# karfly/learnable-triangulation-pytorch

Hardware: NVIDIA H100
Metric: volumetric samples/sec (4-view 384x384, 64^3 grid) (higher is better)
Workload: dtype fp16x3 (split-fp16 operands, 3 wgmma products per term, fp32 accumulate)

## Files before the change

### learnable-triangulation-pytorch_b200/csrc/conv_tc.cu

```cuda
#include "tc_common.cuh"
#include "conv_tc_params.cuh"
#include <stdlib.h>
#include <string.h>

namespace lt {

constexpr int kTcThreads = 384;

struct TcUnit {
  int m, n0, z, q_begin, nchunks;
};
__device__ __forceinline__ TcUnit tc_unit(const TcParams& p, int u, int m_tiles, int nchunks_all) {
  TcUnit w;
  const int n = u % p.n_tiles;
  u /= p.n_tiles;
  w.m = u % m_tiles;
  w.z = u / m_tiles;
  w.n0 = n * p.Nt;
  w.q_begin = (int)(((long)w.z * nchunks_all) / p.splits);
  w.nchunks = (int)(((long)(w.z + 1) * nchunks_all) / p.splits) - w.q_begin;
  return w;
}
__device__ __forceinline__ void tc_tile_origin(const TcParams& p, int t, int& ow0, int& oh0, int& od0, int& nb0) {
  ow0 = (t % p.tw) * p.bw; t /= p.tw;
  oh0 = (t % p.th) * p.bh; t /= p.th;
  od0 = (t % p.td) * p.bd;
  nb0 = (t / p.td) * p.bn;
}

constexpr int kSlabBytes = 128 * 128;
__host__ __device__ constexpr int tc_epi_bytes(int nt, int splits) { return (nt >= 32 && splits == 1) ? nt / 32 * kSlabBytes : 0; }

__device__ __forceinline__ void epi_slab(const TcParams& p, int co, int& g, int& c) {
  g = p.n_maps > 1 ? co / p.oc : 0;
  const int ch = co - g * p.oc;
  c = p.out_format == LT_FMT_F32 ? ch : 2 * ch;
}

__device__ __forceinline__ uint32_t sw128(int row, int b) {
  return (uint32_t)(row * 128 + ((((b >> 4) ^ row) & 7) << 4) + (b & 15));
}

template <int NT>
__global__ void __launch_bounds__(kTcThreads, 1) conv_tc_kernel(const __grid_constant__ CUtensorMap tmA,
                                                                const __grid_constant__ CUtensorMap tmB,
                                                                const __grid_constant__ TcEpiMaps tmE, const TcParams p) {
  extern __shared__ uint8_t smem_raw[];
  uint8_t* smem = reinterpret_cast<uint8_t*>((reinterpret_cast<uintptr_t>(smem_raw) + 1023) & ~(uintptr_t)1023);
  constexpr int kStage = kATileBytes + NT * 128;
  const int epi_bytes = tc_epi_bytes(NT, p.splits);
  const bool staged = epi_bytes > 0;
  uint8_t* ebuf = smem + (size_t)p.stages * kStage;
  uint64_t* full = reinterpret_cast<uint64_t*>(ebuf + epi_bytes);
  uint64_t* empty = full + p.stages;
  uint64_t* efull = empty + p.stages;
  uint64_t* edone = efull + 1;

  const int wg = __shfl_sync(0xffffffffu, (int)(threadIdx.x >> 7), 0);
  const int lane = threadIdx.x & 31;
  const int m_tiles = p.tw * p.th * p.td * p.tn;
  const int units = m_tiles * p.n_tiles * p.splits;
  const int nchunks_all = p.KD * p.KH * p.KW * p.CB;

  if (threadIdx.x == 0) {
    for (int s = 0; s < p.stages; ++s) { mbar_init(&full[s], 1); mbar_init(&empty[s], 2); }
    mbar_init(efull, 1);
    mbar_init(edone, 256);
    fence_barrier_init();
    prefetch_tmap(&tmA);
    prefetch_tmap(&tmB);
  }
  __syncthreads();

  if (wg == 0) {
    regs_release_producer();
    if (staged && threadIdx.x == 32) {
      uint32_t eph = 0;
      for (int u = blockIdx.x; u < units; u += gridDim.x) {
        const TcUnit w = tc_unit(p, u, m_tiles, nchunks_all);
        int ow0, oh0, od0, nb0;
        tc_tile_origin(p, w.m, ow0, oh0, od0, nb0);
        bulk_wait_read0();
        if (p.residual != LT_RES_NONE) {
          mbar_expect_tx(efull, (uint32_t)epi_bytes);
          for (int sl = 0; sl < NT / 32; ++sl) {
            int g, c;
            epi_slab(p, w.n0 + 32 * sl, g, c);
            tma_load_5d(ebuf + sl * kSlabBytes, &tmE.res[g], efull, c, ow0, oh0, od0, nb0);
          }
        } else {
          mbar_arrive_local(efull);
        }
        mbar_wait(edone, eph);
        eph ^= 1u;
        for (int sl = 0; sl < NT / 32; ++sl) {
          int g, c;
          epi_slab(p, w.n0 + 32 * sl, g, c);
          tma_store_5d(&tmE.out[g], ebuf + sl * kSlabBytes, c, ow0, oh0, od0, nb0);
        }
        bulk_commit();
      }
      bulk_wait0();
    }
    if (threadIdx.x < 32) {
      int s = 0;
      uint32_t ph = 0;
      for (int u = blockIdx.x; u < units; u += gridDim.x) {
        const TcUnit w = tc_unit(p, u, m_tiles, nchunks_all);
        int ow0, oh0, od0, nb0;
        tc_tile_origin(p, w.m, ow0, oh0, od0, nb0);
        int tap = w.q_begin / p.CB, cb = w.q_begin - tap * p.CB;
        int kw = tap % p.KW, kh = (tap / p.KW) % p.KH, kd = tap / (p.KW * p.KH);
        const int ax = ow0 * p.sw - p.pw, ay = oh0 * p.sh - p.ph, az = od0 * p.sd - p.pd, bn0 = w.n0 * p.b_nmul;
        for (int q = 0, qa = w.q_begin; q < w.nchunks; ++q, ++qa) {
          mbar_wait(&empty[s], ph ^ 1u);
          uint8_t* a_dst = smem + (size_t)s * kStage;
          if (elect_one()) {
            mbar_expect_tx(&full[s], (uint32_t)kStage);
            tma_load_5d(a_dst, &tmA, &full[s], cb * 64, ax + kw, ay + kh, az + kd, nb0);
            tma_load_2d(a_dst + kATileBytes, &tmB, &full[s], qa * p.b_step0, qa * p.b_step1 + bn0);
          }
          __syncwarp();
          if (++cb == p.CB) { cb = 0; if (++kw == p.KW) { kw = 0; if (++kh == p.KH) { kh = 0; ++kd; } } }
          if (++s == p.stages) { s = 0; ph ^= 1u; }
        }
      }
    }
    return;
  }

  regs_claim_consumer();
  const int g = wg - 1;
  float d1[NT / 2], d2[NT / 2];
#pragma unroll
  for (int i = 0; i < NT / 2; ++i) { d1[i] = 0.f; d2[i] = 0.f; }
  const int r0 = g * 64 + ((threadIdx.x >> 5) & 3) * 16 + (lane >> 2);
  const int c2 = 2 * (lane & 3);
  const uint32_t ring0 = smem_u32(smem);
  int s = 0;
  uint32_t ph = 0, eph = 0;
  for (int u = blockIdx.x; u < units; u += gridDim.x) {
    const TcUnit w = tc_unit(p, u, m_tiles, nchunks_all);
    int prev = -1;
    for (int q = 0; q < w.nchunks; ++q) {
      mbar_wait(&full[s], ph);
      const uint32_t a_addr = ring0 + (uint32_t)(s * kStage) + (uint32_t)(g * 64 * 128);
      const uint32_t b_addr = ring0 + (uint32_t)(s * kStage) + kATileBytes;
      const uint64_t ad = make_sw128_desc(a_addr), bd = make_sw128_desc(b_addr);
      const uint32_t acc = (q == 0) ? 0u : 1u;
      wg_fence();
      if (p.terms == 3) {
        wgmma_f16<NT>(d1, ad, bd, acc);
        wgmma_f16<NT>(d1, ad + 2, bd + 2, 1u);
        wgmma_f16<NT>(d2, ad, bd + 4, acc);
        wgmma_f16<NT>(d2, ad + 2, bd + 6, 1u);
        wgmma_f16<NT>(d2, ad + 4, bd, 1u);
        wgmma_f16<NT>(d2, ad + 6, bd + 2, 1u);
      } else if (p.terms == 1) {
        wgmma_f16<NT>(d1, ad, bd, acc);
        wgmma_f16<NT>(d1, ad + 2, bd + 2, 1u);
      } else {
        wgmma_f16<NT>(d1, ad, bd, acc);
        wgmma_f16<NT>(d1, ad + 2, bd + 2, 1u);
        wgmma_f16<NT>(d1, ad + 4, bd + 4, 1u);
        wgmma_f16<NT>(d1, ad + 6, bd + 6, 1u);
      }
      wg_commit();
      wg_wait<1>();
      if (prev >= 0 && (threadIdx.x & 127) == 0) mbar_arrive_local(&empty[prev]);
      prev = s;
      if (++s == p.stages) { s = 0; ph ^= 1u; }
    }
    wg_wait<0>();
    if (prev >= 0 && (threadIdx.x & 127) == 0) mbar_arrive_local(&empty[prev]);
    wg_fence_regs(d1);
    wg_fence_regs(d2);

    if (p.splits > 1) {
#pragma unroll
      for (int h = 0; h < 2; ++h) {
        float* wrow = p.ws + (((size_t)w.z * m_tiles + w.m) * 128 + r0 + 8 * h) * p.ws_ld + w.n0;
#pragma unroll
        for (int i = 0; i < NT / 8; ++i) {
          const int k = 4 * i + 2 * h;
          const float v0 = (p.terms == 3) ? fmaf(d2[k], kLoInv, d1[k]) : d1[k];
          const float v1 = (p.terms == 3) ? fmaf(d2[k + 1], kLoInv, d1[k + 1]) : d1[k + 1];
          *reinterpret_cast<float2*>(wrow + 8 * i + c2) = make_float2(v0, v1);
        }
      }
      continue;
    }
    if constexpr (NT >= 32) {
      mbar_wait(efull, eph);
      eph ^= 1u;
      const uint32_t e0 = smem_u32(ebuf);
      auto fc_ok = [&](int co) {
        int ch;
        long pix;
        epilogue_target(p, co, 0, ch, pix);
        return ch < p.FC;
      };
      float2 sc = make_float2(0.f, 0.f), sh = sc;
      if (fc_ok(w.n0 + c2)) {
        sc = __ldg(reinterpret_cast<const float2*>(p.scale + w.n0 + c2));
        sh = __ldg(reinterpret_cast<const float2*>(p.shift + w.n0 + c2));
      }
#pragma unroll
      for (int i = 0; i < NT / 8; ++i) {
        const int co = w.n0 + 8 * i + c2;
        const bool ok = fc_ok(co);
        float2 sc_next = sc, sh_next = sh;
        if (i + 1 < NT / 8 && fc_ok(co + 8)) {
          sc_next = __ldg(reinterpret_cast<const float2*>(p.scale + co + 8));
          sh_next = __ldg(reinterpret_cast<const float2*>(p.shift + co + 8));
        }
        const uint32_t slab = e0 + (uint32_t)((i >> 2) * kSlabBytes);
        const int cc = 8 * (i & 3) + c2;
#pragma unroll
        for (int h = 0; h < 2 && ok; ++h) {
          const int row = r0 + 8 * h;
          const int k = 4 * i + 2 * h;
          float v0 = (p.terms == 3) ? fmaf(d2[k], kLoInv, d1[k]) : d1[k];
          float v1 = (p.terms == 3) ? fmaf(d2[k + 1], kLoInv, d1[k + 1]) : d1[k + 1];
          v0 = fmaf(v0, sc.x, sh.x);
          v1 = fmaf(v1, sc.y, sh.y);
          if (p.out_format == LT_FMT_F32) {
            const uint32_t a = slab + sw128(row, 4 * cc);
            float2 r = make_float2(0.f, 0.f);
            if (p.residual != LT_RES_NONE) r = lds_f2(a);
            if (p.residual == LT_RES_BEFORE_RELU) { v0 += r.x; v1 += r.y; }
            if (p.relu) { v0 = fmaxf(v0, 0.f); v1 = fmaxf(v1, 0.f); }
            if (p.residual == LT_RES_AFTER_RELU) { v0 += r.x; v1 += r.y; }
            sts_f2(a, make_float2(v0, v1));
          } else {
            const uint32_t ahi = slab + sw128(row, 2 * cc), alo = slab + sw128(row, 64 + 2 * cc);
            float2 r = make_float2(0.f, 0.f);
            if (p.residual != LT_RES_NONE) {
              const uint32_t rh = lds32(ahi), rl = lds32(alo);
              const float2 a = __half22float2(*reinterpret_cast<const __half2*>(&rh));
              const float2 b = __half22float2(*reinterpret_cast<const __half2*>(&rl));
              r = make_float2(fmaf(b.x, kLoInv, a.x), fmaf(b.y, kLoInv, a.y));
            }
            if (p.residual == LT_RES_BEFORE_RELU) { v0 += r.x; v1 += r.y; }
            if (p.relu) { v0 = fmaxf(v0, 0.f); v1 = fmaxf(v1, 0.f); }
            if (p.residual == LT_RES_AFTER_RELU) { v0 += r.x; v1 += r.y; }
            uint32_t hi2, lo2;
            split_s32x2(v0, v1, hi2, lo2);
            sts32(ahi, hi2);
            sts32(alo, lo2);
          }
        }
        sc = sc_next;
        sh = sh_next;
      }
      fence_proxy_async();
      mbar_arrive_local(edone);
    } else {
      int ow0, oh0, od0, nb0;
      tc_tile_origin(p, w.m, ow0, oh0, od0, nb0);
#pragma unroll
      for (int h = 0; h < 2; ++h) {
        int r_ = r0 + 8 * h;
        const int dw = r_ % p.bw; r_ /= p.bw;
        const int dh = r_ % p.bh; r_ /= p.bh;
        const int dd = r_ % p.bd; r_ /= p.bd;
        const int ow = ow0 + dw, oh = oh0 + dh, od = od0 + dd, nb = nb0 + r_;
        if (!(ow < p.OW && oh < p.OH && od < p.OD && nb < p.N)) continue;
        const long opix = (((long)nb * p.FD + (od * p.osd + p.ood)) * p.FH + (oh * p.osh + p.ooh)) * p.FW + (ow * p.osw + p.oow);
        conv_epilogue_row<NT>(p, d1, d2, h, opix, w.n0, c2);
      }
    }
  }
}

typedef CUresult (*EncodeTiledFn)(CUtensorMap*, CUtensorMapDataType, cuuint32_t, void*, const cuuint64_t*, const cuuint64_t*,
                                  const cuuint32_t*, const cuuint32_t*, CUtensorMapInterleave, CUtensorMapSwizzle,
                                  CUtensorMapL2promotion, CUtensorMapFloatOOBfill);

static EncodeTiledFn encode_fn() {
  static EncodeTiledFn fn = nullptr;
  if (!fn) {
    void* ptr = nullptr;
    cudaDriverEntryPointQueryResult qres;
    if (cudaGetDriverEntryPoint("cuTensorMapEncodeTiled", &ptr, cudaEnableDefault, &qres) == cudaSuccess &&
        qres == cudaDriverEntryPointSuccess)
      fn = reinterpret_cast<EncodeTiledFn>(ptr);
  }
  return fn;
}

struct MapKey {
  const void* base;
  int rank, swizzle, f32;
  uint64_t dims[5], strides[4];
  uint32_t box[5], es[5];
};
struct MapSlot {
  bool used = false;
  MapKey key;
  CUtensorMap map;
};

int make_map(CUtensorMap* map, const void* base, int rank, const uint64_t* dims, const uint64_t* strides_bytes,
             const uint32_t* box, const uint32_t* estrides, int swizzle128, int f32) {
  EncodeTiledFn fn = encode_fn();
  if (!fn) return fail(LT_ERR_CUDA, "cuTensorMapEncodeTiled entry point not available");
  MapKey key;
  memset(&key, 0, sizeof(key));
  key.base = base; key.rank = rank; key.swizzle = swizzle128; key.f32 = f32;
  for (int i = 0; i < rank; ++i) { key.dims[i] = dims[i]; key.box[i] = box[i]; key.es[i] = estrides ? estrides[i] : 1; }
  for (int i = 0; i + 1 < rank; ++i) key.strides[i] = strides_bytes[i];
  uint64_t h = 1469598103934665603ull;
  const unsigned char* kb = reinterpret_cast<const unsigned char*>(&key);
  for (size_t i = 0; i < sizeof(key); ++i) { h ^= kb[i]; h *= 1099511628211ull; }
  static thread_local MapSlot cache[256];
  MapSlot& slot = cache[(h ^ (h >> 29)) & 255];
  if (slot.used && memcmp(&slot.key, &key, sizeof(key)) == 0) {
    *map = slot.map;
    return LT_OK;
  }
  cuuint64_t gd[5], gs[4];
  cuuint32_t bx[5], es[5];
  for (int i = 0; i < rank; ++i) { gd[i] = dims[i]; bx[i] = box[i]; es[i] = estrides ? estrides[i] : 1; }
  for (int i = 0; i + 1 < rank; ++i) gs[i] = strides_bytes[i];
  CUresult r = fn(map, f32 ? CU_TENSOR_MAP_DATA_TYPE_FLOAT32 : CU_TENSOR_MAP_DATA_TYPE_FLOAT16, (cuuint32_t)rank, const_cast<void*>(base), gd, gs, bx, es,
                  CU_TENSOR_MAP_INTERLEAVE_NONE,
                  swizzle128 == 1 ? CU_TENSOR_MAP_SWIZZLE_128B : (swizzle128 == 2 ? CU_TENSOR_MAP_SWIZZLE_64B : CU_TENSOR_MAP_SWIZZLE_NONE),
                  CU_TENSOR_MAP_L2_PROMOTION_L2_128B, CU_TENSOR_MAP_FLOAT_OOB_FILL_NONE);
  if (r != CUDA_SUCCESS) return fail(LT_ERR_CUDA, "cuTensorMapEncodeTiled failed with CUresult %d", (int)r);
  slot.used = true;
  slot.key = key;
  slot.map = *map;
  return LT_OK;
}

static int pow2_ceil(int v) { int p = 1; while (p < v) p <<= 1; return p; }

static void pick_box(int OW, int OH, int OD, int N, int* box) {
  double best = 1e300;
  for (int bw = 1; bw <= 128; bw <<= 1)
    for (int bh = 1; bw * bh <= 128; bh <<= 1)
      for (int bd = 1; bw * bh * bd <= 128; bd <<= 1) {
        const int bn = 128 / (bw * bh * bd);
        if (bw > pow2_ceil(OW) || bh > pow2_ceil(OH) || bd > pow2_ceil(OD) || bn > pow2_ceil(N)) continue;
        const double padded = (double)ceil_div(OW, bw) * bw * ceil_div(OH, bh) * bh * (double)ceil_div(OD, bd) * bd * ceil_div(N, bn) * bn;
        const double score = padded * (1.0 + 1e-3 / bw);
        if (score < best) { best = score; box[0] = bw; box[1] = bh; box[2] = bd; box[3] = bn; }
      }
  if (best == 1e300) { box[0] = pow2_ceil(OW) > 128 ? 128 : pow2_ceil(OW); box[1] = box[2] = 1; box[3] = 128 / box[0]; }
}

__global__ void __launch_bounds__(256) splitk_reduce_kernel(const TcParams p, long m_tiles, int coutp) {
  const int c4 = coutp >> 2;
  const long total = m_tiles * 128 * c4;
  for (long i = (long)blockIdx.x * blockDim.x + threadIdx.x; i < total; i += (long)gridDim.x * blockDim.x) {
    const int co = (int)(i % c4) * 4;
    const long tr = i / c4;
    const int row = (int)(tr % 128);
    long t = tr / 128;
    const int twi = (int)(t % p.tw); t /= p.tw;
    const int thi = (int)(t % p.th); t /= p.th;
    const int tdi = (int)(t % p.td); t /= p.td;
    const int tni = (int)t;
    int r_ = row;
    const int dw = r_ % p.bw; r_ /= p.bw;
    const int dh = r_ % p.bh; r_ /= p.bh;
    const int dd = r_ % p.bd; r_ /= p.bd;
    const int ow = twi * p.bw + dw, oh = thi * p.bh + dh, od = tdi * p.bd + dd, nb = tni * p.bn + r_;
    if (!(ow < p.OW && oh < p.OH && od < p.OD && nb < p.N) || co >= p.FC) continue;
    const long opix = (((long)nb * p.FD + (od * p.osd + p.ood)) * p.FH + (oh * p.osh + p.ooh)) * p.FW + (ow * p.osw + p.oow);
    float4 a = make_float4(0.f, 0.f, 0.f, 0.f);
    for (int z = 0; z < p.splits; ++z) {
      const float4 v = *reinterpret_cast<const float4*>(p.ws + ((size_t)z * m_tiles * 128 + tr) * p.ws_ld + co);
      a.x += v.x; a.y += v.y; a.z += v.z; a.w += v.w;
    }
    const float4 sc = __ldg(reinterpret_cast<const float4*>(p.scale + co));
    const float4 sh = __ldg(reinterpret_cast<const float4*>(p.shift + co));
    float4 o = make_float4(fmaf(a.x, sc.x, sh.x), fmaf(a.y, sc.y, sh.y), fmaf(a.z, sc.z, sh.z), fmaf(a.w, sc.w, sh.w));
    float4 rr = make_float4(0.f, 0.f, 0.f, 0.f);
    if (p.residual != LT_RES_NONE) {
      if (p.out_format == LT_FMT_F32) rr = *reinterpret_cast<const float4*>(reinterpret_cast<const float*>(p.res) + opix * p.FC + co);
      else rr = load_s32x4(reinterpret_cast<const sh_t*>(p.res) + opix * 2 * p.FC, co);
    }
    if (p.residual == LT_RES_BEFORE_RELU) { o.x += rr.x; o.y += rr.y; o.z += rr.z; o.w += rr.w; }
    if (p.relu) { o.x = fmaxf(o.x, 0.f); o.y = fmaxf(o.y, 0.f); o.z = fmaxf(o.z, 0.f); o.w = fmaxf(o.w, 0.f); }
    if (p.residual == LT_RES_AFTER_RELU) { o.x += rr.x; o.y += rr.y; o.z += rr.z; o.w += rr.w; }
    if (p.out_format == LT_FMT_F32) *reinterpret_cast<float4*>(reinterpret_cast<float*>(p.out) + opix * p.FC + co) = o;
    else store_s32x4(reinterpret_cast<sh_t*>(p.out) + opix * 2 * p.FC, co, o);
  }
}

static int out_groups(const lt_conv_desc* d) {
  const int g = (d->ogd > 1 ? d->ogd : 1) * (d->ogh > 1 ? d->ogh : 1) * (d->ogw > 1 ? d->ogw : 1);
  return g;
}

static int pick_nt(int CoutP) {
  for (int nt = 128; nt > 16; nt >>= 1)
    if (CoutP % nt == 0) return nt;
  return 16;
}

template <int NT>
static int launch_nt(const CUtensorMap& tmA, const CUtensorMap& tmB, const TcEpiMaps& tmE, const TcParams& p, dim3 grid, size_t smem,
                     cudaStream_t st) {
  static DeviceOnce configured;
  if (configured.first()) {
    cudaError_t e = cudaFuncSetAttribute(conv_tc_kernel<NT>, cudaFuncAttributeMaxDynamicSharedMemorySize, (int)(227 * 1024));
    if (e != cudaSuccess) return fail(LT_ERR_CUDA, "conv_tc: cudaFuncSetAttribute: %s", cudaGetErrorString(e));
  }
  conv_tc_kernel<NT><<<grid, kTcThreads, smem, st>>>(tmA, tmB, tmE, p);
  cudaError_t e = cudaGetLastError();
  if (e != cudaSuccess) return fail(LT_ERR_CUDA, "conv_tc_kernel: %s", cudaGetErrorString(e));
  return LT_OK;
}

static double tc_model_clocks(long tiles, int chunks, int nt, int splits, int sm) {
  const long units = tiles * splits;
  const long grid = units < sm ? units : sm;
  const long waves = (units + grid - 1) / grid;
  const double chunk = fmax(12.0 * 64.0 * nt / 128.0, (kATileBytes + nt * 128.0) / 30.0);
  const double epilogue = 128.0 * nt * 4.0 / 30.0;
  double t = (double)waves * ((double)ceil_div(chunks, splits) * chunk + epilogue);
  if (splits > 1) t += 7000.0 + (double)tiles * 128 * nt * 4.0 * (splits + 2) / 1500.0;
  return t;
}

static void tc_plan(long m_tiles, int n_tiles, int nt, int chunks, int terms, int n_maps, int splitk, size_t ws_bytes, int sm,
                    int* splits_out, int* grid_out) {
  const long tiles = m_tiles * n_tiles;
  int best = 1;
  if (splitk && terms != 0 && n_maps == 1) {
    const size_t per_split = (size_t)tiles * 128 * nt * sizeof(float);
    double best_t = tc_model_clocks(tiles, chunks, nt, 1, sm);
    for (int s = 2; s <= chunks / 4 && (size_t)s * per_split <= ws_bytes; ++s) {
      const double t = tc_model_clocks(tiles, chunks, nt, s, sm);
      if (t < best_t) { best_t = t; best = s; }
    }
  }
  const long units = tiles * best;
  *splits_out = best;
  *grid_out = (int)(units < sm ? units : sm);
}

static int group_extent(int n, int F, int off, int ph, int os) {
  const int e = (F - off - ph + os - 1) / os;
  return e < n ? e : n;
}

static int make_epi_maps(const TcParams& p, TcEpiMaps* m) {
  const int f32 = p.out_format == LT_FMT_F32;
  const uint64_t rowb = (uint64_t)p.FC * 4;
  const uint64_t str[4] = {rowb * p.osw, rowb * p.FW * p.osh, rowb * p.FW * p.FH * p.osd, rowb * p.FW * p.FH * p.FD};
  const uint32_t bx[5] = {f32 ? 32u : 64u, (uint32_t)p.bw, (uint32_t)p.bh, (uint32_t)p.bd, (uint32_t)p.bn};
  for (int g = 0; g < p.n_maps; ++g) {
    const int ga = g / (p.gh * p.gw), gb = (g / p.gw) % p.gh, gc = g % p.gw;
    const int ew = group_extent(p.OW, p.FW, p.oow, gc, p.osw), eh = group_extent(p.OH, p.FH, p.ooh, gb, p.osh),
              ed = group_extent(p.OD, p.FD, p.ood, ga, p.osd);
    LT_REQUIRE(ew > 0 && eh > 0 && ed > 0, "conv_tc: output group %d lies outside the %dx%dx%d output tensor", g, p.FD, p.FH, p.FW);
    const uint64_t dims[5] = {(uint64_t)(f32 ? p.FC : 2 * p.FC), (uint64_t)ew, (uint64_t)eh, (uint64_t)ed, (uint64_t)p.N};
    const long pix0 = ((long)(p.ood + ga) * p.FH + p.ooh + gb) * p.FW + p.oow + gc;
    int rc = make_map(&m->out[g], static_cast<const uint8_t*>(p.out) + pix0 * rowb, 5, dims, str, bx, nullptr, 1, f32);
    if (rc) return rc;
    if (p.residual == LT_RES_NONE) continue;
    rc = make_map(&m->res[g], static_cast<const uint8_t*>(p.res) + pix0 * rowb, 5, dims, str, bx, nullptr, 1, f32);
    if (rc) return rc;
  }
  return LT_OK;
}

constexpr int kTcSmemBudget = 224 * 1024;

static int launch_tc(const CUtensorMap& tmA, const CUtensorMap& tmB, TcParams& p, int n_tiles, cudaStream_t st, void* ws = nullptr,
                     size_t ws_bytes = 0) {
  const long m_tiles = (long)p.tw * p.th * p.td * p.tn;
  int splits, grid;
  tc_plan(m_tiles, n_tiles, p.Nt, p.KD * p.KH * p.KW * p.CB, p.terms, p.n_maps, ws ? opts().tc_splitk : 0, ws_bytes, sm_count(),
          &splits, &grid);
  p.splits = splits;
  p.ws = reinterpret_cast<float*>(ws);
  p.ws_ld = n_tiles * p.Nt;
  p.n_tiles = n_tiles;
  const int stage_bytes = kATileBytes + p.Nt * 128;
  const int epi_bytes = tc_epi_bytes(p.Nt, splits);
  int stages = (kTcSmemBudget - epi_bytes) / stage_bytes;
  if (stages > 8) stages = 8;
  p.stages = stages;
  const size_t smem = (size_t)stages * stage_bytes + epi_bytes + (2 * stages + 2) * 8 + 1024;
  TcEpiMaps tmE{};
  int rc;
  if (epi_bytes) {
    rc = make_epi_maps(p, &tmE);
    if (rc) return rc;
  }
  switch (p.Nt) {
    case 128: rc = launch_nt<128>(tmA, tmB, tmE, p, dim3(grid), smem, st); break;
    case 64: rc = launch_nt<64>(tmA, tmB, tmE, p, dim3(grid), smem, st); break;
    case 32: rc = launch_nt<32>(tmA, tmB, tmE, p, dim3(grid), smem, st); break;
    case 16: rc = launch_nt<16>(tmA, tmB, tmE, p, dim3(grid), smem, st); break;
    default: return fail(LT_ERR_INVALID, "conv_tc: unsupported N tile %d", p.Nt);
  }
  if (rc) return rc;
  if (splits > 1) {
    const long total = m_tiles * 128 * (p.ws_ld / 4);
    long blocks = (total + 255) / 256;
    if (blocks > 4L * sm_count()) blocks = 4L * sm_count();
    splitk_reduce_kernel<<<(unsigned)blocks, 256, 0, st>>>(p, m_tiles, p.ws_ld);
    cudaError_t e = cudaGetLastError();
    if (e != cudaSuccess) return fail(LT_ERR_CUDA, "splitk_reduce_kernel: %s", cudaGetErrorString(e));
  }
  return LT_OK;
}

void fill_params(const lt_conv_desc* d, TcParams& p, int CB, int CoutP, int Nt, int terms, const float* scale, const float* shift,
                        const void* residual, void* out) {
  p.OW = d->OW; p.OH = d->OH; p.OD = d->OD; p.N = d->N;
  int box[4];
  pick_box(d->OW, d->OH, d->OD, d->N, box);
  p.bw = box[0]; p.bh = box[1]; p.bd = box[2]; p.bn = box[3];
  p.tw = ceil_div(d->OW, p.bw); p.th = ceil_div(d->OH, p.bh); p.td = ceil_div(d->OD, p.bd); p.tn = ceil_div(d->N, p.bn);
  p.KW = d->KW; p.KH = d->KH; p.KD = d->KD; p.pw = d->pw; p.ph = d->ph; p.pd = d->pd;
  p.sw = d->sw; p.sh = d->sh; p.sd = d->sd;
  p.CB = CB; p.b_step0 = 0; p.b_step1 = CoutP; p.b_nmul = 1; p.Nt = Nt; p.terms = terms;
  p.FC = d->FC; p.FD = d->FD; p.FH = d->FH; p.FW = d->FW;
  p.osd = d->osd; p.osh = d->osh; p.osw = d->osw; p.ood = d->ood; p.ooh = d->ooh; p.oow = d->oow;
  p.relu = d->relu; p.residual = d->residual; p.out_format = d->out_format;
  p.scale = scale; p.shift = shift; p.res = residual; p.out = out;
  p.splits = 1; p.ws = nullptr; p.ws_ld = 0; p.stages = 0; p.n_tiles = 1;
  p.n_maps = out_groups(d);
  p.oc = p.n_maps > 1 ? d->Cout / p.n_maps : CoutP;
  p.gh = d->ogh > 1 ? d->ogh : 1; p.gw = d->ogw > 1 ? d->ogw : 1;
}

int make_in_map(CUtensorMap* tmA, const lt_conv_desc* d, int bw, int bh, int bd, int bn, const void* in) {
  const uint64_t rowb = (uint64_t)d->Cin * 2 * 2;
  const uint64_t dims[5] = {(uint64_t)d->Cin * 2, (uint64_t)d->IW, (uint64_t)d->IH, (uint64_t)d->ID, (uint64_t)d->N};
  const uint64_t str[4] = {rowb, rowb * d->IW, rowb * d->IW * d->IH, rowb * d->IW * d->IH * d->ID};
  const uint32_t es[5] = {1, (uint32_t)d->sw, (uint32_t)d->sh, (uint32_t)d->sd, 1};
  uint32_t bx[5] = {64, (uint32_t)bw, (uint32_t)bh, (uint32_t)bd, (uint32_t)bn};
  for (int i = 1; i <= 3; ++i) bx[i] = (bx[i] - 1) * es[i] + 1;
  LT_REQUIRE(bx[1] <= 256 && bx[2] <= 256 && bx[3] <= 256, "conv_tc: strided box exceeds 256");
  return make_map(tmA, in, 5, dims, str, bx, es, 1);
}

static bool groups_ok(const lt_conv_desc* d, int CoutP) {
  const int G = out_groups(d);
  return d->Cout % G == 0 && (d->Cout / G) % 32 == 0 && d->Cout / G == d->FC && CoutP == d->Cout && G <= kMaxOutMaps;
}

int conv_tc_fwd_terms(const lt_conv_desc* d, const void* in, const void* weight, const float* scale, const float* shift,
                      const void* residual, void* out, int terms, void* stream) {
  LT_REQUIRE(d->in_format == LT_FMT_S32, "conv_tc: input must be split-fp16");
  LT_REQUIRE(d->Cin % 32 == 0, "conv_tc: Cin=%d must be a multiple of 32", d->Cin);
  LT_REQUIRE(d->FC % 4 == 0 && (d->out_format == LT_FMT_F32 || d->FC % 32 == 0), "conv_tc: bad output channel stride %d", d->FC);
  LT_REQUIRE((reinterpret_cast<uintptr_t>(out) | reinterpret_cast<uintptr_t>(residual)) % 16 == 0,
             "conv_tc: out and residual must be 16-byte aligned (TMA global addresses)");
  const int CoutP = (d->Cout + 15) & ~15;
  const int CB = d->Cin / 32;
  const int taps = d->KD * d->KH * d->KW;
  const int Nt = pick_nt(CoutP);
  TcParams p;
  fill_params(d, p, CB, CoutP, Nt, terms, scale, shift, residual, out);
  if (p.n_maps > 1)
    LT_REQUIRE(groups_ok(d, CoutP), "conv_tc: grouped output needs Cout / groups == FC, a multiple of 32");
  CUtensorMap tmA, tmB;
  int rc = make_in_map(&tmA, d, p.bw, p.bh, p.bd, p.bn, in);
  if (rc) return rc;
  {
    const uint64_t dims[2] = {64, (uint64_t)taps * CB * CoutP};
    const uint64_t str[1] = {128};
    const uint32_t bx[2] = {64, (uint32_t)Nt};
    rc = make_map(&tmB, weight, 2, dims, str, bx, nullptr, 1);
    if (rc) return rc;
  }
  return launch_tc(tmA, tmB, p, CoutP / Nt, (cudaStream_t)stream, d->workspace, d->workspace_bytes);
}

__global__ void __launch_bounds__(256) pack_weights_kernel(const float* __restrict__ w, sh_t* __restrict__ out,
                                                           int taps, int Cin, int Cout, int CoutP) {
  const int CB = Cin / 32;
  const long total = (long)taps * CB * CoutP * 32;
  for (long i = (long)blockIdx.x * blockDim.x + threadIdx.x; i < total; i += (long)gridDim.x * blockDim.x) {
    const int j = (int)(i % 32);
    long r = i / 32;
    const int n = (int)(r % CoutP); r /= CoutP;
    const int cb = (int)(r % CB);
    const int tap = (int)(r / CB);
    const float v = (n < Cout) ? w[((long)tap * Cin + cb * 32 + j) * Cout + n] : 0.0f;
    sh_t hi, lo;
    split_s32(v, hi, lo);
    sh_t* rowp = out + ((((long)tap * CB + cb) * CoutP + n) << 6);
    rowp[j] = hi;
    rowp[32 + j] = lo;
  }
}

__global__ void ones_zeros_kernel(float* ones, float* zeros, int n) {
  const int i = blockIdx.x * blockDim.x + threadIdx.x;
  if (i < n) { ones[i] = 1.0f; zeros[i] = 0.0f; }
}

}

using namespace lt;

extern "C" int lt_conv_tc_plan(const lt_conv_desc* d, int sm_count, int splitk, lt_conv_tc_launch_plan* plan) {
  LT_REQUIRE(d && plan && sm_count > 0, "conv_tc_plan: bad arguments");
  LT_REQUIRE(d->Cin % 32 == 0 && d->Cout > 0, "conv_tc_plan: Cin=%d must be a multiple of 32", d->Cin);
  const int CoutP = (d->Cout + 15) & ~15;
  int box[4];
  pick_box(d->OW, d->OH, d->OD, d->N, box);
  plan->nt = pick_nt(CoutP);
  plan->m_tiles = ceil_div(d->OW, box[0]) * ceil_div(d->OH, box[1]) * ceil_div(d->OD, box[2]) * ceil_div(d->N, box[3]);
  plan->n_tiles = CoutP / plan->nt;
  plan->chunks = d->KD * d->KH * d->KW * (d->Cin / 32);
  tc_plan(plan->m_tiles, plan->n_tiles, plan->nt, plan->chunks, 3, out_groups(d), d->workspace ? splitk : 0, d->workspace_bytes,
          sm_count, &plan->splits, &plan->grid);
  return LT_OK;
}

extern "C" size_t lt_conv_tc_weight_bytes(int taps, int Cin, int Cout) {
  const int CoutP = (Cout + 15) & ~15;
  return (size_t)taps * (Cin / 32) * CoutP * 128;
}

extern "C" int lt_conv_tc_pack_weights(const float* w, void* packed, int taps, int Cin, int Cout, void* stream) {
  LT_REQUIRE(w && packed, "conv_tc_pack_weights: null pointer");
  LT_REQUIRE(Cin % 32 == 0 && taps > 0 && Cout > 0, "conv_tc_pack_weights: bad sizes");
  const int CoutP = (Cout + 15) & ~15;
  const long total = (long)taps * (Cin / 32) * CoutP * 32;
  long blocks = (total + 255) / 256;
  if (blocks > 65535) blocks = 65535;
  pack_weights_kernel<<<(unsigned)blocks, 256, 0, (cudaStream_t)stream>>>(w, reinterpret_cast<sh_t*>(packed), taps, Cin, Cout, CoutP);
  LT_CHECK_LAUNCH("pack_weights_kernel");
  return LT_OK;
}

extern "C" int lt_tc_gemm_selftest(const void* a, const void* b, float* d, int M, int N, int K, int variant, void* stream) {
  LT_REQUIRE(a && b && d, "tc_gemm_selftest: null pointer");
  LT_REQUIRE(M > 0 && N % 16 == 0 && N >= 16 && K % 64 == 0, "tc_gemm_selftest: need N %% 16 == 0, K %% 64 == 0");
  (void)variant;
  const int Nt = pick_nt(N);
  float* ones = d + (size_t)M * N;
  float* zeros = ones + N;
  ones_zeros_kernel<<<ceil_div(N, 256), 256, 0, (cudaStream_t)stream>>>(ones, zeros, N);
  TcParams p;
  p.OW = M; p.OH = 1; p.OD = 1; p.N = 1;
  p.bw = 128; p.bh = 1; p.bd = 1; p.bn = 1;
  p.tw = ceil_div(M, 128); p.th = 1; p.td = 1; p.tn = 1;
  p.KW = p.KH = p.KD = 1; p.pw = p.ph = p.pd = 0; p.sw = p.sh = p.sd = 1;
  p.CB = K / 64; p.b_step0 = 64; p.b_step1 = 0; p.b_nmul = 1; p.Nt = Nt; p.terms = 0;
  p.FC = N; p.FD = 1; p.FH = 1; p.FW = M; p.osd = p.osh = p.osw = 1; p.ood = p.ooh = p.oow = 0;
  p.relu = 0; p.residual = LT_RES_NONE; p.out_format = LT_FMT_F32;
  p.scale = ones; p.shift = zeros; p.res = nullptr; p.out = d;
  p.n_maps = 1; p.oc = N; p.gh = p.gw = 1;
  p.splits = 1; p.ws = nullptr; p.ws_ld = 0; p.n_tiles = 1;
  CUtensorMap tmA, tmB;
  {
    const uint64_t dims[5] = {(uint64_t)K, (uint64_t)M, 1, 1, 1};
    const uint64_t str[4] = {(uint64_t)K * 2, (uint64_t)K * 2 * M, (uint64_t)K * 2 * M, (uint64_t)K * 2 * M};
    const uint32_t bx[5] = {64, 128, 1, 1, 1};
    int rc = make_map(&tmA, a, 5, dims, str, bx, nullptr, 1);
    if (rc) return rc;
  }
  {
    const uint64_t dims[2] = {(uint64_t)K, (uint64_t)N};
    const uint64_t str[1] = {(uint64_t)K * 2};
    const uint32_t bx[2] = {64, (uint32_t)Nt};
    int rc = make_map(&tmB, b, 2, dims, str, bx, nullptr, 1);
    if (rc) return rc;
  }
  return launch_tc(tmA, tmB, p, N / Nt, (cudaStream_t)stream);
}
```

### learnable-triangulation-pytorch_b200/csrc/conv_tc_params.cuh

```cuda
#pragma once
#include "tc_common.cuh"

namespace lt {

struct TcParams {
  int OW, OH, OD, N;
  int bw, bh, bd, bn;
  int tw, th, td, tn;
  int KW, KH, KD, pw, ph, pd;
  int sw, sh, sd;
  int CB;
  int b_step0, b_step1;
  int b_nmul;
  int Nt, stages, terms;
  int FC, FD, FH, FW, osd, osh, osw, ood, ooh, oow, relu, residual, out_format;
  const float* scale;
  const float* shift;
  const void* res;
  void* out;
  int splits, ws_ld;
  float* ws;
  int n_tiles;
  int oc, n_maps;
  int gh, gw;
};

constexpr int kMaxOutMaps = 8;

struct TcEpiMaps {
  CUtensorMap out[kMaxOutMaps];
  CUtensorMap res[kMaxOutMaps];
};

constexpr int kATileBytes = 128 * 128;

__device__ __forceinline__ void epilogue_target(const TcParams& p, int co, long opix, int& ch, long& pix) {
  ch = co;
  pix = opix;
  if (p.n_maps > 1) {
    const int mi = ch / p.oc;
    ch -= mi * p.oc;
    pix += ((long)(mi / (p.gh * p.gw)) * p.FH + (mi / p.gw) % p.gh) * p.FW + mi % p.gw;
  }
}

template <int NT>
__device__ __forceinline__ float2 epilogue_residual(const TcParams& p, int ch, long pix) {
  if (p.residual == LT_RES_NONE || ch >= p.FC) return make_float2(0.f, 0.f);
  if (p.out_format == LT_FMT_F32) return *reinterpret_cast<const float2*>(reinterpret_cast<const float*>(p.res) + pix * p.FC + ch);
  const sh_t* rp = reinterpret_cast<const sh_t*>(p.res) + pix * 2 * p.FC + s32_off(ch);
  const float2 a = __half22float2(*reinterpret_cast<const __half2*>(rp));
  const float2 b = __half22float2(*reinterpret_cast<const __half2*>(rp + 32));
  return make_float2(fmaf(b.x, kLoInv, a.x), fmaf(b.y, kLoInv, a.y));
}

template <int NT>
__device__ __forceinline__ void conv_epilogue_row(const TcParams& p, const float (&d1)[NT / 2], const float (&d2)[NT / 2], int h,
                                                  long opix, int n0, int c2) {
  static_assert(NT <= 32, "wider tiles would not hold the hoisted residual beside their accumulators");
  float2 rr[NT / 8];
#pragma unroll
  for (int i = 0; i < NT / 8; ++i) {
    int ch;
    long pix;
    epilogue_target(p, n0 + 8 * i + c2, opix, ch, pix);
    rr[i] = epilogue_residual<NT>(p, ch, pix);
  }
#pragma unroll
  for (int i = 0; i < NT / 8; ++i) {
    const int k = 4 * i + 2 * h;
    const int co = n0 + 8 * i + c2;
    int ch;
    long pix;
    epilogue_target(p, co, opix, ch, pix);
    if (ch >= p.FC) continue;
    float v0 = (p.terms == 3) ? fmaf(d2[k], kLoInv, d1[k]) : d1[k];
    float v1 = (p.terms == 3) ? fmaf(d2[k + 1], kLoInv, d1[k + 1]) : d1[k + 1];
    const float2 sc = __ldg(reinterpret_cast<const float2*>(p.scale + co));
    const float2 sh = __ldg(reinterpret_cast<const float2*>(p.shift + co));
    v0 = fmaf(v0, sc.x, sh.x);
    v1 = fmaf(v1, sc.y, sh.y);
    const float2 r = rr[i];
    if (p.residual == LT_RES_BEFORE_RELU) { v0 += r.x; v1 += r.y; }
    if (p.relu) { v0 = fmaxf(v0, 0.f); v1 = fmaxf(v1, 0.f); }
    if (p.residual == LT_RES_AFTER_RELU) { v0 += r.x; v1 += r.y; }
    if (p.out_format == LT_FMT_F32) {
      *reinterpret_cast<float2*>(reinterpret_cast<float*>(p.out) + pix * p.FC + ch) = make_float2(v0, v1);
    } else {
      uint32_t hi2, lo2;
      split_s32x2(v0, v1, hi2, lo2);
      sh_t* op = reinterpret_cast<sh_t*>(p.out) + pix * 2 * p.FC + s32_off(ch);
      *reinterpret_cast<uint32_t*>(op) = hi2;
      *reinterpret_cast<uint32_t*>(op + 32) = lo2;
    }
  }
}

void fill_params(const lt_conv_desc* d, TcParams& p, int CB, int CoutP, int Nt, int terms, const float* scale, const float* shift,
                 const void* residual, void* out);
int make_in_map(CUtensorMap* tmA, const lt_conv_desc* d, int bw, int bh, int bd, int bn, const void* in);

}
```

Measured before the change: 193.9.

## Double-buffer the TMA epilogue staging buffer for short-K conv units

```diff
diff --git a/learnable-triangulation-pytorch_b200/csrc/conv_tc.cu b/learnable-triangulation-pytorch_b200/csrc/conv_tc.cu
--- a/learnable-triangulation-pytorch_b200/csrc/conv_tc.cu
+++ b/learnable-triangulation-pytorch_b200/csrc/conv_tc.cu
@@ -50,11 +50,12 @@
   constexpr int kStage = kATileBytes + NT * 128;
   const int epi_bytes = tc_epi_bytes(NT, p.splits);
   const bool staged = epi_bytes > 0;
+  const int nbuf = p.ebufs;
   uint8_t* ebuf = smem + (size_t)p.stages * kStage;
-  uint64_t* full = reinterpret_cast<uint64_t*>(ebuf + epi_bytes);
+  uint64_t* full = reinterpret_cast<uint64_t*>(ebuf + (size_t)nbuf * epi_bytes);
   uint64_t* empty = full + p.stages;
   uint64_t* efull = empty + p.stages;
-  uint64_t* edone = efull + 1;
+  uint64_t* edone = efull + 2;
 
   const int wg = __shfl_sync(0xffffffffu, (int)(threadIdx.x >> 7), 0);
   const int lane = threadIdx.x & 31;
@@ -64,8 +65,7 @@
 
   if (threadIdx.x == 0) {
     for (int s = 0; s < p.stages; ++s) { mbar_init(&full[s], 1); mbar_init(&empty[s], 2); }
-    mbar_init(efull, 1);
-    mbar_init(edone, 256);
+    for (int b = 0; b < 2; ++b) { mbar_init(&efull[b], 1); mbar_init(&edone[b], 256); }
     fence_barrier_init();
     prefetch_tmap(&tmA);
     prefetch_tmap(&tmB);
@@ -75,30 +75,44 @@
   if (wg == 0) {
     regs_release_producer();
     if (staged && threadIdx.x == 32) {
-      uint32_t eph = 0;
-      for (int u = blockIdx.x; u < units; u += gridDim.x) {
+      auto load_residual = [&](int u, int b) {
         const TcUnit w = tc_unit(p, u, m_tiles, nchunks_all);
         int ow0, oh0, od0, nb0;
         tc_tile_origin(p, w.m, ow0, oh0, od0, nb0);
-        bulk_wait_read0();
+        uint8_t* eb = ebuf + (size_t)b * epi_bytes;
         if (p.residual != LT_RES_NONE) {
-          mbar_expect_tx(efull, (uint32_t)epi_bytes);
+          mbar_expect_tx(&efull[b], (uint32_t)epi_bytes);
           for (int sl = 0; sl < NT / 32; ++sl) {
             int g, c;
             epi_slab(p, w.n0 + 32 * sl, g, c);
-            tma_load_5d(ebuf + sl * kSlabBytes, &tmE.res[g], efull, c, ow0, oh0, od0, nb0);
+            tma_load_5d(eb + sl * kSlabBytes, &tmE.res[g], &efull[b], c, ow0, oh0, od0, nb0);
           }
         } else {
-          mbar_arrive_local(efull);
-        }
-        mbar_wait(edone, eph);
-        eph ^= 1u;
+          mbar_arrive_local(&efull[b]);
+        }
+      };
+      if ((int)blockIdx.x < units) load_residual(blockIdx.x, 0);
+      int i = 0;
+      for (int u = blockIdx.x; u < units; u += gridDim.x, ++i) {
+        const int b = i % nbuf, next = u + gridDim.x;
+        if (nbuf == 2 && next < units) {
+          bulk_wait_read0();
+          load_residual(next, b ^ 1);
+        }
+        const TcUnit w = tc_unit(p, u, m_tiles, nchunks_all);
+        int ow0, oh0, od0, nb0;
+        tc_tile_origin(p, w.m, ow0, oh0, od0, nb0);
+        mbar_wait(&edone[b], (uint32_t)(i / nbuf) & 1u);
         for (int sl = 0; sl < NT / 32; ++sl) {
           int g, c;
           epi_slab(p, w.n0 + 32 * sl, g, c);
-          tma_store_5d(&tmE.out[g], ebuf + sl * kSlabBytes, c, ow0, oh0, od0, nb0);
+          tma_store_5d(&tmE.out[g], ebuf + (size_t)b * epi_bytes + sl * kSlabBytes, c, ow0, oh0, od0, nb0);
         }
         bulk_commit();
+        if (nbuf == 1 && next < units) {
+          bulk_wait_read0();
+          load_residual(next, 0);
+        }
       }
       bulk_wait0();
     }
@@ -138,8 +152,8 @@
   const int c2 = 2 * (lane & 3);
   const uint32_t ring0 = smem_u32(smem);
   int s = 0;
-  uint32_t ph = 0, eph = 0;
-  for (int u = blockIdx.x; u < units; u += gridDim.x) {
+  uint32_t ph = 0;
+  for (int u = blockIdx.x, i = 0; u < units; u += gridDim.x, ++i) {
     const TcUnit w = tc_unit(p, u, m_tiles, nchunks_all);
     int prev = -1;
     for (int q = 0; q < w.nchunks; ++q) {
@@ -191,9 +205,9 @@
       continue;
     }
     if constexpr (NT >= 32) {
-      mbar_wait(efull, eph);
-      eph ^= 1u;
-      const uint32_t e0 = smem_u32(ebuf);
+      const int b = i % nbuf;
+      mbar_wait(&efull[b], (uint32_t)(i / nbuf) & 1u);
+      const uint32_t e0 = smem_u32(ebuf + (size_t)b * epi_bytes);
       auto fc_ok = [&](int co) {
         int ch;
         long pix;
@@ -254,7 +268,7 @@
         sh = sh_next;
       }
       fence_proxy_async();
-      mbar_arrive_local(edone);
+      mbar_arrive_local(&edone[b]);
     } else {
       int ow0, oh0, od0, nb0;
       tc_tile_origin(p, w.m, ow0, oh0, od0, nb0);
@@ -470,6 +484,7 @@
 }
 
 constexpr int kTcSmemBudget = 224 * 1024;
+constexpr int kTcShortK = 4;
 
 static int launch_tc(const CUtensorMap& tmA, const CUtensorMap& tmB, TcParams& p, int n_tiles, cudaStream_t st, void* ws = nullptr,
                      size_t ws_bytes = 0) {
@@ -483,10 +498,12 @@
   p.n_tiles = n_tiles;
   const int stage_bytes = kATileBytes + p.Nt * 128;
   const int epi_bytes = tc_epi_bytes(p.Nt, splits);
-  int stages = (kTcSmemBudget - epi_bytes) / stage_bytes;
+  const int unit_chunks = ceil_div(p.KD * p.KH * p.KW * p.CB, splits);
+  p.ebufs = (epi_bytes && unit_chunks <= kTcShortK && (kTcSmemBudget - 2 * epi_bytes) / stage_bytes >= 3) ? 2 : 1;
+  int stages = (kTcSmemBudget - p.ebufs * epi_bytes) / stage_bytes;
   if (stages > 8) stages = 8;
   p.stages = stages;
-  const size_t smem = (size_t)stages * stage_bytes + epi_bytes + (2 * stages + 2) * 8 + 1024;
+  const size_t smem = (size_t)stages * stage_bytes + (size_t)p.ebufs * epi_bytes + (2 * stages + 4) * 8 + 1024;
   TcEpiMaps tmE{};
   int rc;
   if (epi_bytes) {
@@ -526,7 +543,7 @@
   p.osd = d->osd; p.osh = d->osh; p.osw = d->osw; p.ood = d->ood; p.ooh = d->ooh; p.oow = d->oow;
   p.relu = d->relu; p.residual = d->residual; p.out_format = d->out_format;
   p.scale = scale; p.shift = shift; p.res = residual; p.out = out;
-  p.splits = 1; p.ws = nullptr; p.ws_ld = 0; p.stages = 0; p.n_tiles = 1;
+  p.splits = 1; p.ws = nullptr; p.ws_ld = 0; p.stages = 0; p.n_tiles = 1; p.ebufs = 1;
   p.n_maps = out_groups(d);
   p.oc = p.n_maps > 1 ? d->Cout / p.n_maps : CoutP;
   p.gh = d->ogh > 1 ? d->ogh : 1; p.gw = d->ogw > 1 ? d->ogw : 1;
@@ -654,7 +671,7 @@
   p.relu = 0; p.residual = LT_RES_NONE; p.out_format = LT_FMT_F32;
   p.scale = ones; p.shift = zeros; p.res = nullptr; p.out = d;
   p.n_maps = 1; p.oc = N; p.gh = p.gw = 1;
-  p.splits = 1; p.ws = nullptr; p.ws_ld = 0; p.n_tiles = 1;
+  p.splits = 1; p.ws = nullptr; p.ws_ld = 0; p.n_tiles = 1; p.ebufs = 1;
   CUtensorMap tmA, tmB;
   {
     const uint64_t dims[5] = {(uint64_t)K, (uint64_t)M, 1, 1, 1};
diff --git a/learnable-triangulation-pytorch_b200/csrc/conv_tc_params.cuh b/learnable-triangulation-pytorch_b200/csrc/conv_tc_params.cuh
--- a/learnable-triangulation-pytorch_b200/csrc/conv_tc_params.cuh
+++ b/learnable-triangulation-pytorch_b200/csrc/conv_tc_params.cuh
@@ -23,6 +23,7 @@
   int n_tiles;
   int oc, n_maps;
   int gh, gw;
+  int ebufs;
 };
 
 constexpr int kMaxOutMaps = 8;
```

After: 199.2, median of 6. 1.03x the previous value.
